# sdmiller/cpu_tsdf

Measured on NVIDIA H100. Metric: integrateCloud frames/s @ 640x480 into 2048^3, higher is better.
Workload: dtype f32

## Files before the change

cpu_tsdf_b200/csrc/brick_kernels.cuh:

```cuda
#pragma once
#include "tsdf_core.cuh"
#include "obs_fast.cuh"

namespace b2 {

struct QNode
{
  int x, y, z;
  int slot, idx;
  int kind;
  int child_base;
  int rc;
};

struct FrameRec
{
  Frame f;
  float pl[6][4];
  int cset;
  int timing;
  int pad_[2];
  unsigned long long kt[2];
};
__device__ __forceinline__ void pdl_launch_dependents () { asm volatile ("griddepcontrol.launch_dependents;" ::: "memory"); }
// ... 218 lines not shown
        Obs oc = observe (p, f, ch.cx, ch.cy, ch.cz, ch.size);
        rc = visit_fresh_leaf (p, f, ch, oc, cnt);
      }
      const unsigned nonneg = __ballot_sync (0xffffffffu, lane < 8 && rc >= 0);
      upd += cnt.n_updates; vis += cnt.n_visits;
      if (nonneg) return 1;
      if (lane == 0) atomicAnd (sw, ~m);
      if (lane < 8) reset_node (p, ch);
      __syncwarp ();
    }
  }
  int rc = 0;
  if (lane == 0) { bool updated; rc = leaf_update (p, f, n, o, updated); upd += updated; }
  return __shfl_sync (0xffffffffu, rc, 0);
}

constexpr int FRESH_RECS = 128;
struct CoopWarp
{
  __device__ __forceinline__ int lane () const { return threadIdx.x & 31; }
  __device__ __forceinline__ int nlanes () const { return 32; }
  __device__ __forceinline__ void sync () const { __syncwarp (); }
};
__device__ __noinline__ int leaf_visit_warp_bfs (const Params& p, const Frame& f, const NodePos& n, FreshRec* rec, int* counter,
                                                 unsigned long long& upd, unsigned long long& vis)
{
  const int lane = threadIdx.x & 31;
  Obs o = observe (p, f, n.cx, n.cy, n.cz, n.size);
  if (!o.valid) return 0;
  if (o.near_ && n.size > p.finest_size)
  {
    uint32_t m; uint32_t* sw = split_word (p, n, m);
    int cs = -1;
    if (lane == 0) cs = children_slot (p, n, true);
    cs = __shfl_sync (0xffffffffu, cs, 0);
    if (cs >= 0)
    {
      if (lane == 0) atomicOr (sw, m);
      __syncwarp ();
      Counters cnt; cnt.n_updates = 0; cnt.n_visits = 0;
      const bool stays = fresh_children_bfs (p, f, n, cs, rec, FRESH_RECS, counter, CoopWarp (), cnt);
      upd += cnt.n_updates; vis += cnt.n_visits;
      if (stays) return 1;
      if (lane == 0) atomicAnd (sw, ~m);
      if (lane < 8) reset_node (p, rec[lane].n);
      __syncwarp ();
    }
  }
  int rc = 0;
  if (lane == 0) { bool updated; rc = leaf_update (p, f, n, o, updated); upd += updated; }
  return __shfl_sync (0xffffffffu, rc, 0);
}

__device__ __noinline__ int leaf_visit_groups (const Params& p, const Frame& f, const NodePos& n, bool active,
                                               unsigned long long& upd, unsigned long long& vis)
{
  const int lane = threadIdx.x & 31, sub = lane & 7, g = lane >> 3;
  const unsigned gmask = 0xFFu << (8 * g);
  Obs o; o.valid = false; o.near_ = false; o.u = o.v = 0; o.d_new = 0.f;
  if (active) o = observe (p, f, n.cx, n.cy, n.cz, n.size);
  const bool live = active && o.valid;
  const bool want_split = live && o.near_ && n.size > p.finest_size;
  uint32_t m = 0; uint32_t* sw = nullptr;
  int cs = -1;
  if (want_split) { sw = split_word (p, n, m); if (sub == 0) cs = children_slot (p, n, true); }
  cs = __shfl_sync (0xffffffffu, cs, 8 * g);
  const bool split = want_split && cs >= 0;
  if (split && sub == 0) atomicOr (sw, m);
  __syncwarp ();
  Counters cnt; cnt.n_updates = 0; cnt.n_visits = 0;
  int crc = -1;
  NodePos ch = n;
  if (split)
  {
    ch = make_child (p, n, sub, cs);
    Obs oc = observe (p, f, ch.cx, ch.cy, ch.cz, ch.size);
    crc = visit_fresh_leaf (p, f, ch, oc, cnt);
  }
  const unsigned nonneg = __ballot_sync (0xffffffffu, split && crc >= 0) & gmask;
  upd += cnt.n_updates; vis += cnt.n_visits;
  if (split && !nonneg)
  {
    if (sub == 0) atomicAnd (sw, ~m);
    reset_node (p, ch);
  }
  __syncwarp ();
  int rc = 0;
  if (split && nonneg) rc = 1;
  else if (live && sub == 0) { bool updated; rc = leaf_update (p, f, n, o, updated); upd += updated; }
  return __shfl_sync (0xffffffffu, rc, 8 * g);
}
__device__ __forceinline__ void leaf_visit_slow_lanes (const Params& p, const Frame& f, bool slow, const NodePos& n, int t1, int& rc,
                                                       unsigned long long& upd, unsigned long long& vis)
{
  const int lane = threadIdx.x & 31, g = lane >> 3;
  uint32_t sm = __ballot_sync (0xffffffffu, slow);
  while (sm)
  {
    int srcs[4];
#pragma unroll
    for (int k = 0; k < 4; ++k) { srcs[k] = sm ? __ffs (sm) - 1 : -1; if (sm) sm &= sm - 1; }
    int src = srcs[0]; if (g == 1) src = srcs[1]; if (g == 2) src = srcs[2]; if (g == 3) src = srcs[3];
    const int from = src >= 0 ? src : 0;
    NodePos q;
    q.level = __shfl_sync (0xffffffffu, n.level, from); q.x = __shfl_sync (0xffffffffu, n.x, from); q.y = __shfl_sync (0xffffffffu, n.y, from); q.z = __shfl_sync (0xffffffffu, n.z, from);
    q.cx = __shfl_sync (0xffffffffu, n.cx, from); q.cy = __shfl_sync (0xffffffffu, n.cy, from); q.cz = __shfl_sync (0xffffffffu, n.cz, from);
    q.size = __shfl_sync (0xffffffffu, n.size, from); q.slot = t1; q.idx = __shfl_sync (0xffffffffu, n.idx, from);
    __threadfence_block ();
    const int r = leaf_visit_groups (p, f, q, src >= 0, upd, vis);
#pragma unroll
    for (int k = 0; k < 4; ++k) { const int rk = __shfl_sync (0xffffffffu, r, 8 * k); if (lane == srcs[k]) rc = rk; }
  }
}

__device__ __forceinline__ void path_center (const float* c0, float off, int k, int j, float* c)
{
  float x = c0[0], y = c0[1], z = c0[2];
  for (int l = k - 1; l >= 0; --l)
  {
    int cc = (j >> (3 * l)) & 7;
    x = (cc & 4) ? fadd (x, off) : fsub (x, off);
    y = (cc & 2) ? fadd (y, off) : fsub (y, off);
    z = (cc & 1) ? fadd (z, off) : fsub (z, off);
    off *= 0.5f;
  }
  c[0] = x; c[1] = y; c[2] = z;
}

constexpr int TOP_THREADS = 256;
constexpr int TOP_NODES = 585;
struct CellTop
{
  int t1slot, nblk;
  unsigned char kind[592];
  signed char rc[592];
  float dnew[73];
  int uv[73];
};
struct TopSmem
{
  float2 dw[BRICK_NODES];
  uchar4 rgb[BRICK_NODES];
  float o_dnew[TOP_NODES];
  int o_uv[TOP_NODES];
  uint32_t o_bgra[TOP_NODES];
  unsigned char o_flags[592];
  unsigned char kind[592];
  signed char rc[592];
  unsigned char dirty[592];
  uint32_t split[BRICK_SPLIT_WORDS];
  uint32_t split_old[BRICK_SPLIT_WORDS];
  QNode cell;
  int t1slot, root_interior;
  float c0[3];
};

__device__ __forceinline__ void top_kj (int f, int& k, int& j)
{ if (f == 0) { k = 0; j = 0; } else if (f < 9) { k = 1; j = f - 1; } else if (f < 73) { k = 2; j = f - 9; } else { k = 3; j = f - 73; } }

template <bool COLOR>
__global__ void __launch_bounds__ (TOP_THREADS) k_celltop_down (Params p, const FrameRec* __restrict__ fr, QNode* __restrict__ cells, int* __restrict__ d_count,
                                                               QNode* __restrict__ gq, CellTop* __restrict__ tops, int cell_cap,
                                                               int* __restrict__ blist, int bl_stride, unsigned long long* __restrict__ stats,
                                                               int SL, int qslot, int static_count)
{
  __shared__ __align__ (16) TopSmem S;
  __shared__ Frame s_f_;
  __shared__ float s_pl_[6][4];
  const int tid = threadIdx.x, lane = tid & 31;
  pdl_launch_dependents ();
  {
    const int* src_ = reinterpret_cast<const int*> (&fr->f); int* dst_ = reinterpret_cast<int*> (&s_f_);
    for (int w_ = tid; w_ < (int) (sizeof (Frame) / sizeof (int)); w_ += TOP_THREADS) dst_[w_] = src_[w_];
    if (tid < 24) s_pl_[tid >> 2][tid & 3] = fr->pl[tid >> 2][tid & 3];
  }
  int* const cnt_ = d_count + 16 * fr->cset;
  __syncthreads ();
  pdl_wait ();
  const Frame& f = s_f_;
  unsigned long long upd = 0, vis = 0;
  int count = qslot >= 0 ? cnt_[qslot] : static_count;
  if (count > cell_cap) { if (tid == 0 && blockIdx.x == 0) raise_err (p, ERR_QUEUE_FULL); count = cell_cap; }
  const int cell_lvl = p.C - SL;
  const float sizeC = level_size (p, SL);
  const float off1 = sizeC * 0.25f;
  const double thr[4] = { near_threshold (sizeC), near_threshold (sizeC * 0.5f), near_threshold (sizeC * 0.25f), near_threshold (sizeC * 0.125f) };
  const float thrf[4] = { float_at_least (thr[0]), float_at_least (thr[1]), float_at_least (thr[2]), float_at_least (thr[3]) };
// ... 29 lines not shown
      if (cell_lvl > 0)
      {
        kind = KIND_OLD;
        slot = find_brick (p, 1, cell.x, cell.y, cell.z);
        if (slot < 0) { raise_err (p, ERR_MISSING_BRICK); kind = KIND_DONE; }
      }
      else
      {
        NodePos nc; nc.level = SL; nc.x = cell.x; nc.y = cell.y; nc.z = cell.z; nc.cx = c0[0]; nc.cy = c0[1]; nc.cz = c0[2]; nc.size = sizeC; nc.slot = cell.slot; nc.idx = cell.idx;
        uint32_t m; uint32_t* sw = split_word (p, nc, m);
        vis++;
        if (*sw & m) { kind = KIND_OLD; slot = find_brick (p, 1, cell.x, cell.y, cell.z); if (slot < 0) { raise_err (p, ERR_MISSING_BRICK); kind = KIND_DONE; } }
        else
        {
          Obs o = observe_thr (p, f, c0[0], c0[1], c0[2], thr[0]);
          if (o.valid)
          {
            if (o.near_) { slot = find_or_insert_brick (p, 1, cell.x, cell.y, cell.z); if (slot >= 0) { kind = KIND_NEW; atomicOr (sw, m); } }
            else { bool u_; rc = leaf_update (p, f, nc, o, u_); upd += u_; }
          }
        }
        if (kind == KIND_DONE) cells[ci].rc = rc;
      }
      S.root_interior = kind; S.t1slot = slot;
      S.kind[0] = (unsigned char) kind; S.rc[0] = (signed char) rc;
    }
    __syncthreads ();
    const int t1 = S.t1slot;
    CellTop* top = tops + ci;
    if (S.root_interior == KIND_DONE)
    {
      if (tid == 0) { top->t1slot = -1; top->nblk = 0; top->kind[0] = KIND_DONE; top->rc[0] = S.rc[0]; }
      continue;
    }
    float2* gdw = p.nodes + (size_t) t1 * BRICK_NODES;
    uchar4* grgb = COLOR ? p.rgb + (size_t) t1 * BRICK_NODES : nullptr;
    uint32_t* gsw = p.split + (size_t) t1 * BRICK_SPLIT_WORDS;
    {
      const float4* g4 = reinterpret_cast<const float4*> (gdw);
      float4* s4 = reinterpret_cast<float4*> (S.dw);
      for (int i = tid; i < BRICK_NODES / 2; i += TOP_THREADS) s4[i] = g4[i];
      if (COLOR)
      {
        const uint4* gc = reinterpret_cast<const uint4*> (grgb);
        uint4* sc = reinterpret_cast<uint4*> (S.rgb);
        for (int i = tid; i < BRICK_NODES / 4; i += TOP_THREADS) sc[i] = gc[i];
// ... 68 lines not shown
          if (cls == c) blist[(size_t) c * bl_stride + b + __popc (mask & ((1u << lane) - 1))] = ci * STRIDE + 73 + j3;
        }
      }
    }
    for (int n = 1 + tid; n < TOP_NODES; n += TOP_THREADS)
      if (S.dirty[n]) { gdw[n - 1] = S.dw[n - 1]; if (COLOR) grgb[n - 1] = S.rgb[n - 1]; }
    if (tid < BRICK_SPLIT_WORDS && S.split[tid] != S.split_old[tid]) gsw[tid] = S.split[tid];
    for (int n = tid; n < 592; n += TOP_THREADS) { top->kind[n] = n < TOP_NODES ? S.kind[n] : 0; top->rc[n] = n < TOP_NODES ? S.rc[n] : 0; }
    for (int n = tid; n < 73; n += TOP_THREADS) { top->dnew[n] = S.o_dnew[n]; top->uv[n] = S.o_uv[n]; }
    if (tid == 0) { top->t1slot = t1; top->nblk = 0; }
  }
  __syncwarp ();
  warp_add_stats (stats, upd, vis);
}

__device__ __forceinline__ int top_fallthrough_new (const Params& p, const Frame& f, const NodePos& n, float dnew, int uv, unsigned long long& upd)
{
  Obs o; o.valid = true; o.near_ = true; o.d_new = dnew; o.u = uv & 0xFFFF; o.v = uv >> 16;
  bool u_; int rc = leaf_update (p, f, n, o, u_); upd += u_;
  return rc;
}

template <bool COLOR>
__global__ void __launch_bounds__ (128) k_celltop_up (Params gp, const FrameRec* __restrict__ fr, QNode* __restrict__ cells, const int* __restrict__ d_count,
                                                      const QNode* __restrict__ gq, const CellTop* __restrict__ tops, int cell_cap,
                                                      unsigned long long* __restrict__ stats, int SL, int qslot, int static_count)
{
  __shared__ Params sp_;
  __shared__ Frame sf_;
  __shared__ FreshRec s_rec[4][FRESH_RECS];
  __shared__ int s_cnt[4];
  pdl_launch_dependents ();
  {
    const int* s1 = reinterpret_cast<const int*> (&gp); int* d1 = reinterpret_cast<int*> (&sp_);
    for (int w = threadIdx.x; w < (int) (sizeof (Params) / sizeof (int)); w += blockDim.x) d1[w] = s1[w];
    const int* s2 = reinterpret_cast<const int*> (&fr->f); int* d2 = reinterpret_cast<int*> (&sf_);
    for (int w = threadIdx.x; w < (int) (sizeof (Frame) / sizeof (int)); w += blockDim.x) d2[w] = s2[w];
  }
  __syncthreads ();
  pdl_wait ();
  const Params& p = sp_;
  const Frame& f = sf_;
  const int lane = threadIdx.x & 31;
  const int warp = (blockIdx.x * blockDim.x + threadIdx.x) >> 5, nwarps = (gridDim.x * blockDim.x) >> 5;
  unsigned long long upd = 0, vis = 0;
  int count = qslot >= 0 ? d_count[16 * fr->cset + qslot] : static_count;
  if (count > cell_cap) count = cell_cap;
  if (fr->timing && blockIdx.x == 0 && threadIdx.x == 0 && fr->kt[1] > fr->kt[0])
  { atomicAdd (&stats[5], fr->kt[1] - fr->kt[0]); atomicAdd (&stats[6], 1ull); }
  const float sizeC = level_size (p, SL);
  const float off1 = sizeC * 0.25f;
  const int cell_lvl = p.C - SL;
  constexpr int STRIDE = 585;
  const long long c_entry = clock64 ();
  for (int ci = warp; ci < count; ci += nwarps)
  {
    const long long tc0 = clock64 ();
    int dbg_slow2 = 0, dbg_slow1 = 0, dbg_ft = 0;
    const CellTop* top = tops + ci;
    const int t1 = top->t1slot;
    if (t1 < 0) continue;
    const QNode cell = cells[ci];
    const float c0[3] = { center1d (p, SL, cell.x), center1d (p, SL, cell.y), center1d (p, SL, cell.z) };
    float2* gdw = p.nodes + (size_t) t1 * BRICK_NODES;
    uchar4* grgb = COLOR ? p.rgb + (size_t) t1 * BRICK_NODES : nullptr;
    uint32_t* gsw = p.split + (size_t) t1 * BRICK_SPLIT_WORDS;
    const int kind1 = lane < 8 ? top->kind[1 + lane] : KIND_DONE;
    int kind2[2]; kind2[0] = top->kind[9 + lane]; kind2[1] = top->kind[9 + 32 + lane];
    const uint32_t int1 = __ballot_sync (0xffffffffu, kind1 != KIND_DONE);
    uint32_t int2[2]; int2[0] = __ballot_sync (0xffffffffu, kind2[0] != KIND_DONE); int2[1] = __ballot_sync (0xffffffffu, kind2[1] != KIND_DONE);
    uint32_t nonneg_mine = 0;
    {
      int k3[16], r3[16];
#pragma unroll
      for (int i = 0; i < 16; ++i) { k3[i] = top->kind[73 + lane + 32 * i]; r3[i] = top->rc[73 + lane + 32 * i]; }
#pragma unroll
      for (int i = 0; i < 16; ++i) if (k3[i] != KIND_DONE) r3[i] = gq[(size_t) ci * STRIDE + 73 + lane + 32 * i].rc;
#pragma unroll
      for (int i = 0; i < 16; ++i)
      {
        const int j2 = (lane + 32 * i) >> 3;
        const bool visited = ((j2 < 32 ? int2[0] : int2[1]) >> (j2 & 31)) & 1;
        const uint32_t nn = __ballot_sync (0xffffffffu, visited && r3[i] >= 0);
        if (lane == i) nonneg_mine = nn;
      }
    }
    const long long cA = clock64 ();
    uint32_t nonneg2[2];
#pragma unroll
    for (int i2 = 0; i2 < 2; ++i2)
    {
      const int j2 = lane + 32 * i2;
      const uint32_t nn = __shfl_sync (0xffffffffu, nonneg_mine, (lane >> 2) + 8 * i2);
      int rc = top->rc[9 + j2];
      bool slow = false;
      NodePos n;
      if (kind2[i2] != KIND_DONE)
      {
        if (((nn >> (8 * (lane & 3))) & 0xFFu) != 0 || 2 < cell_lvl) rc = 1;
        else
        {
          atomicAnd (&gsw[1 + (j2 >> 5)], ~(1u << (j2 & 31)));
          for (int c = 0; c < 8; ++c) { gdw[72 + 8 * j2 + c] = make_float2 (-1.f, 0.f); if (COLOR) grgb[72 + 8 * j2 + c] = make_uchar4 (0, 0, 0, 0); }
          float c[3]; path_center (c0, off1, 2, j2, c);
          n.level = SL + 2; n.cx = c[0]; n.cy = c[1]; n.cz = c[2]; n.size = sizeC * 0.25f; n.slot = t1; n.idx = 8 + j2;
          { int lx = 0, ly = 0, lz = 0; for (int q = 1; q >= 0; --q) { int cc = (j2 >> (3 * q)) & 7; lx = (lx << 1) | (cc >> 2); ly = (ly << 1) | ((cc >> 1) & 1); lz = (lz << 1) | (cc & 1); }
            n.x = (cell.x << 2) | lx; n.y = (cell.y << 2) | ly; n.z = (cell.z << 2) | lz; }
          if (kind2[i2] == KIND_NEW) { rc = top_fallthrough_new (p, f, n, top->dnew[9 + j2], top->uv[9 + j2], upd); dbg_ft++; }
          else slow = true;
        }
      }
      dbg_slow2 += __popc (__ballot_sync (0xffffffffu, slow));
      leaf_visit_slow_lanes (p, f, slow, n, t1, rc, upd, vis);
      const bool visited2 = (int1 >> (j2 >> 3)) & 1;
      nonneg2[i2] = __ballot_sync (0xffffffffu, visited2 && rc >= 0);
    }
    const long long cB = clock64 ();
    int rc1 = lane < 8 ? (int) top->rc[1 + lane] : 0;
    {
      bool slow = false;
      NodePos n;
      if (lane < 8 && kind1 != KIND_DONE)
      {
        const uint32_t nn = nonneg2[lane >> 2];
        if (((nn >> (8 * (lane & 3))) & 0xFFu) != 0 || 1 < cell_lvl) rc1 = 1;
        else
        {
          atomicAnd (&gsw[0], ~(1u << lane));
          for (int c = 0; c < 8; ++c) { gdw[8 + 8 * lane + c] = make_float2 (-1.f, 0.f); if (COLOR) grgb[8 + 8 * lane + c] = make_uchar4 (0, 0, 0, 0); }
          float c[3]; path_center (c0, off1, 1, lane, c);
          n.level = SL + 1; n.cx = c[0]; n.cy = c[1]; n.cz = c[2]; n.size = sizeC * 0.5f; n.slot = t1; n.idx = lane;
          n.x = (cell.x << 1) | ((lane >> 2) & 1); n.y = (cell.y << 1) | ((lane >> 1) & 1); n.z = (cell.z << 1) | (lane & 1);
          if (kind1 == KIND_NEW) rc1 = top_fallthrough_new (p, f, n, top->dnew[1 + lane], top->uv[1 + lane], upd);
          else slow = true;
        }
      }
      dbg_slow1 += __popc (__ballot_sync (0xffffffffu, slow));
      leaf_visit_slow_lanes (p, f, slow, n, t1, rc1, upd, vis);
    }
    const uint32_t nonneg1 = __ballot_sync (0xffffffffu, lane < 8 && rc1 >= 0);
    const long long cC = clock64 ();
    int dbg_cell = 0;
    int rc_cell = 1;
    if ((nonneg1 & 0xFFu) == 0 && cell_lvl <= 0)
    {
      dbg_cell = top->kind[0] == KIND_NEW ? 1 : 2;
      NodePos nc; nc.level = SL; nc.x = cell.x; nc.y = cell.y; nc.z = cell.z; nc.cx = c0[0]; nc.cy = c0[1]; nc.cz = c0[2]; nc.size = sizeC; nc.slot = cell.slot; nc.idx = cell.idx;
      if (lane == 0) { uint32_t m; uint32_t* sw = split_word (p, nc, m); atomicAnd (sw, ~m); }
      if (lane < 8) { gdw[lane] = make_float2 (-1.f, 0.f); if (COLOR) grgb[lane] = make_uchar4 (0, 0, 0, 0); }
      __syncwarp ();
      if (top->kind[0] == KIND_NEW) { if (lane == 0) rc_cell = top_fallthrough_new (p, f, nc, top->dnew[0], top->uv[0], upd); rc_cell = __shfl_sync (0xffffffffu, rc_cell, 0); }
      else { __threadfence_block (); rc_cell = leaf_visit_warp_bfs (p, f, nc, s_rec[threadIdx.x >> 5], &s_cnt[threadIdx.x >> 5], upd, vis); }
    }
    if (lane == 0 && cell_lvl <= 0) cells[ci].rc = rc_cell;
    if (p.dbg && lane == 0)
    {
      const long long cD = clock64 ();
      const unsigned long long tag = ((unsigned long long) (dbg_slow2 & 0xFF) << 24) | ((unsigned long long) (dbg_slow1 & 0xF) << 20) | ((unsigned long long) (dbg_cell & 3) << 18) | (unsigned long long) (ci & 0x3FFFF);
      atomicMax (&p.dbg[0], ((unsigned long long) (cD - tc0) << 32) | tag);
      atomicMax (&p.dbg[1], ((unsigned long long) (cA - tc0) << 32) | tag);
      atomicMax (&p.dbg[2], ((unsigned long long) (cB - cA) << 32) | tag);
      atomicMax (&p.dbg[3], ((unsigned long long) (cC - cB) << 32) | tag);
      atomicMax (&p.dbg[4], ((unsigned long long) (cD - cC) << 32) | tag);
      atomicMax (&p.dbg[5], ((unsigned long long) (tc0 - c_entry) << 32) | tag);
      atomicAdd (&p.dbg[6], (unsigned long long) dbg_slow2); atomicAdd (&p.dbg[7], (unsigned long long) dbg_slow1);
      atomicAdd (&p.dbg[8], (unsigned long long) (dbg_cell == 2)); atomicAdd (&p.dbg[9], (unsigned long long) (dbg_cell == 1));
      atomicAdd (&p.dbg[10], 1ull);
    }
  }
  __syncwarp ();
  warp_add_stats (stats, upd, vis);
}

}
```

cpu_tsdf_b200/csrc/engine.cu:

```cuda
#include "../../include/b200tsdf.h"
#include "tsdf_core.cuh"
#include "mc_tables.cuh"
#include "host_math.h"
#include "params_setup.h"
#include "brick_kernels.cuh"
#include "brick_direct.cuh"
#include "organize.cuh"
#include "mesh_sort.h"
#include "host_pack.h"

#include <cuda_runtime.h>
#include <sys/mman.h>
#include <sys/syscall.h>
#include <unistd.h>
#include <algorithm>
#include <cstdio>
#include <cstdlib>
#include <cstring>
#include <string>
#include <type_traits>
#include <unordered_map>
#include <vector>

using namespace b2;
// ... 477 lines not shown
  b200tsdf_config cfg_pending{}, cfg{};
  bool has_volume = false;
  Params p{};
  int device = 0, sm_count = 0;
  cudaStream_t stream = nullptr, copy_stream = nullptr, gather_stream = nullptr;
  size_t pool = 0;
  bool alloc_color = false, alloc_var = false, alloc_norm = false;
  size_t root_n = 0;
  int* d_err = nullptr;
  unsigned char* d_frame[2] = { nullptr, nullptr };
  size_t frame_cap = 0;
  cudaEvent_t ev_copied[2] = { nullptr, nullptr }, ev_consumed[2] = { nullptr, nullptr };
  cudaEvent_t ev_t0 = nullptr, ev_t1 = nullptr, ev_k0 = nullptr, ev_k1 = nullptr;
  uint64_t frame_no = 0;
  int count_set = 0;
  int* d_culled = nullptr; int* d_count = nullptr; unsigned long long* d_stats = nullptr;
  size_t culled_cap = 0;
  bool timed = false;
  bool time_frames = false;
  bool is_empty = true;
  Queues Q{}; int q_levels = 0; QNode* q_mem = nullptr; size_t q_mem_cap = 0;
  int* d_blist = nullptr; int* d_bail = nullptr; size_t blist_cap = 0;
  int cell_cap = 0; QNode* d_cellq = nullptr; size_t cellq_cap = 0; CellTop* d_celltop = nullptr; QNode* d_superq = nullptr;
  bool top_path = false, replayable = false; int sl = 0, nup = 0, super_static = 0;
  bool fast_path = false; int force_general = 0;
  bool use_pdl = true;
  int bd_minb = 6;
  Params* d_params = nullptr;
  unsigned long long* d_dbg = nullptr;
  int* h_err = nullptr;
  FrameRec* d_ring = nullptr; FrameRec* h_ring = nullptr; uint64_t ring_seq = 0;
  cudaEvent_t ev_ring[2] = { nullptr, nullptr };
  FrameRec* d_bring = nullptr; FrameRec* h_bring = nullptr; int bring_half = 0; int bring_seg = 0; bool bring_used[BATCH_SEGS] = {};
  cudaEvent_t ev_bring[BATCH_SEGS] = {};
  cudaEvent_t ev_half_done[2] = { nullptr, nullptr }; bool half_used[2] = { false, false }; FrameRec* batch_recs = nullptr;
  cudaGraphExec_t batch_exec[2][FRAME_RING / 2 + 1] = {};
  void* comm = nullptr; int comm_rank = 0, comm_size = 1;
  unsigned char* d_rows_raw[2] = { nullptr, nullptr }; unsigned char* d_rows_full[2] = { nullptr, nullptr };
  size_t rows_raw_cap = 0, rows_full_cap = 0; int rows_set = 0; bool rows_used[2] = { false, false }; int rows_last_up[2] = { 0, 0 };
  int rows_chunk = 0;
  cudaEvent_t ev_rows_up[2][32] = {}, ev_rows_ready[2][32] = {}, ev_rows_done[2] = { nullptr, nullptr };
  int host_pack = -1;
  int pack_threads = 0;
  b2host::PackPool* pack_pool = nullptr;
  Staging h_pack[2]; size_t pack_cap = 0;
  Staging h_fpack[2];
// ... 217 lines not shown
  if (!h) return;
  cudaSetDevice (h->device);
  if (h->stream) cudaStreamSynchronize (h->stream);
  if (h->copy_stream) cudaStreamSynchronize (h->copy_stream);
  if (h->gather_stream) cudaStreamSynchronize (h->gather_stream);
  free_volume (h);
  cudaFree (h->d_err); cudaFree (h->d_count); cudaFree (h->d_stats); cudaFree (h->d_culled); cudaFree (h->d_scratch);
  cudaFree (h->d_dbg); if (h->h_err) cudaFreeHost (h->h_err);
  cudaFree (h->d_params); cudaFree (h->d_ring); if (h->h_ring) cudaFreeHost (h->h_ring);
  for (int i = 0; i < 2; ++i) if (h->ev_ring[i]) cudaEventDestroy (h->ev_ring[i]);
  drop_batch_graphs (h);
  comm_release (h);
  delete h->pack_pool; h->pack_pool = nullptr;
  for (int i = 0; i < 2; ++i)
  {
    cudaFree (h->d_rows_raw[i]); cudaFree (h->d_rows_full[i]);
    h->h_pack[i].release (); h->h_fpack[i].release ();
    for (int k = 0; k < 32; ++k) { if (h->ev_rows_ready[i][k]) cudaEventDestroy (h->ev_rows_ready[i][k]); if (h->ev_rows_up[i][k]) cudaEventDestroy (h->ev_rows_up[i][k]); }
    if (h->ev_rows_done[i]) cudaEventDestroy (h->ev_rows_done[i]);
  }
  cudaFree (h->d_bring); if (h->h_bring) cudaFreeHost (h->h_bring);
  for (int i = 0; i < BATCH_SEGS; ++i) if (h->ev_bring[i]) cudaEventDestroy (h->ev_bring[i]);
  for (int i = 0; i < 2; ++i) if (h->ev_half_done[i]) cudaEventDestroy (h->ev_half_done[i]);
  cudaFree (h->d_frame[0]); cudaFree (h->d_frame[1]); cudaFree (h->q_mem); cudaFree (h->d_blist); cudaFree (h->d_bail); cudaFree (h->d_cellq); cudaFree (h->d_superq); cudaFree (h->d_celltop);
  for (int i = 0; i < 2; ++i) { if (h->ev_copied[i]) cudaEventDestroy (h->ev_copied[i]); if (h->ev_consumed[i]) cudaEventDestroy (h->ev_consumed[i]); }
  if (h->ev_t0) cudaEventDestroy (h->ev_t0); if (h->ev_t1) cudaEventDestroy (h->ev_t1);
  if (h->ev_k0) cudaEventDestroy (h->ev_k0); if (h->ev_k1) cudaEventDestroy (h->ev_k1);
  if (h->ev_p0) cudaEventDestroy (h->ev_p0); if (h->ev_p1) cudaEventDestroy (h->ev_p1);
  for (int i = 0; i < KRING; ++i) { if (h->kring[i][0]) cudaEventDestroy (h->kring[i][0]); if (h->kring[i][1]) cudaEventDestroy (h->kring[i][1]); }
  if (h->stream) cudaStreamDestroy (h->stream);
  if (h->copy_stream) cudaStreamDestroy (h->copy_stream);
  if (h->gather_stream) cudaStreamDestroy (h->gather_stream);
  std::free (h->mesh_v); std::free (h->mesh_c); std::free (h->leaf_xyz); std::free (h->leaf_ijk);
  delete h;
}

const char* b200tsdf_last_error (const b200tsdf_t* h) { return h ? h->err.c_str () : "null handle"; }

int b200tsdf_set_config (b200tsdf_t* h, const b200tsdf_config* cfg)
{
  if (!h || !cfg) return B200TSDF_EINVAL;
  int dev = h->cfg_pending.device;
  h->cfg_pending = *cfg;
  h->cfg_pending.device = dev;
  std::memcpy (h->cfg.global_transform, cfg->global_transform, sizeof (h->cfg.global_transform));
  return B200TSDF_OK;
}
// ... 63 lines not shown
      cudaFree (h->q_mem); h->q_mem = nullptr; h->q_mem_cap = 0;
      CK (cudaMalloc (&h->q_mem, total * sizeof (QNode)));
      h->q_mem_cap = total;
    }
    size_t off = 0;
    for (int i = 0; i < MAX_QLEVELS; ++i) { h->Q.q[i] = nullptr; h->Q.cap[i] = 0; }
    for (int i = 0; i < h->q_levels; ++i) { h->Q.q[i] = h->q_mem + off; h->Q.cap[i] = (int) caps[i]; off += caps[i]; }
    h->Q.n = h->d_count;
    h->sl = np.L - 6;
    h->nup = std::max (0, h->sl - np.C);
    h->super_static = 0;
    h->top_path = h->fast_path && np.T >= 2 && h->sl >= 0 && !(c.debug_flags & 6);
    if (h->top_path && np.C > h->sl)
    {
      if (np.Rtop != h->sl || h->sl > 4) h->top_path = false;
      else h->super_static = 1 << (3 * h->sl);
    }
    if (h->top_path)
    {
      h->cell_cap = 16384;
      size_t need = (size_t) h->cell_cap * 585;
      if (need > h->cellq_cap)
      {
        cudaFree (h->d_cellq); cudaFree (h->d_celltop); h->d_cellq = nullptr; h->d_celltop = nullptr; h->cellq_cap = 0;
        CK (cudaMalloc (&h->d_cellq, need * sizeof (QNode)));
        CK (cudaMalloc (&h->d_celltop, (size_t) h->cell_cap * sizeof (CellTop)));
        h->cellq_cap = need;
      }
      if (h->super_static && !h->d_superq) CK (cudaMalloc (&h->d_superq, 4096 * sizeof (QNode)));
    }
    h->replayable = h->fast_path;
    size_t bl = h->q_levels ? caps[h->q_levels - 1] : 0;
    if (h->top_path) bl = std::max (bl, (size_t) h->cell_cap * 512);
    if (bl > h->blist_cap)
    {
      cudaFree (h->d_blist); cudaFree (h->d_bail); h->d_blist = h->d_bail = nullptr; h->blist_cap = 0;
      CK (cudaMalloc (&h->d_blist, bl * BL_CLASSES * sizeof (int)));
      CK (cudaMalloc (&h->d_bail, bl * sizeof (int)));
      h->blist_cap = bl;
    }
  }
  Params& p = h->p;
  {
    Params st = p;
    p = np;
    p.work = st.work;
    p.keys = st.keys; p.nodes = st.nodes; p.split = st.split; p.rgb = st.rgb; p.M = st.M; p.ns = st.ns;
    p.root_dw = st.root_dw; p.root_split = st.root_split; p.root_rgb = st.root_rgb; p.root_M = st.root_M; p.root_ns = st.root_ns;
    p.rgbn = st.rgbn; p.root_rgbn = st.root_rgbn;
// ... 53 lines not shown
  {
    const int cull_blocks = (ncells + 255) / 256;
    const bool pdl = h->replayable && h->use_pdl;
    if (pdl) CK (launch_pdl (k_front, dim3 (cull_blocks + (npix + 255) / 256), dim3 (256), s, p, d_rec, cull_blocks, h->d_culled, h->d_count, h->Q.q[0], h->d_stats));
    else k_front<<<cull_blocks + (npix + 255) / 256, 256, 0, s>>> (p, d_rec, cull_blocks, h->d_culled, h->d_count, h->fast_path ? h->Q.q[0] : nullptr, h->d_stats);
  }
  h->launches += 1;
  int kr = -1;
  if (with_events)
  {
    if (h->kring_pending >= KRING) h->drain_kring (KRING / 2);
    kr = h->kring_head;
  }
  if (h->fast_path)
  {
    const int nl = h->q_levels;
    QNode* bq = nullptr;
    if (h->top_path)
    {
      for (int li = 0; li < h->nup; ++li) { k_upper_down<<<h->sm_count * 2, 128, 0, s>>> (p, d_rec, h->Q, li, 0, h->d_blist, h->d_stats); h->launches++; }
      QNode* cells = h->super_static ? h->d_superq : h->Q.q[h->nup];
      const int qslot = h->super_static ? -1 : h->nup;
      auto kd = p.color ? k_celltop_down<true> : k_celltop_down<false>;
      if (h->use_pdl) CK (launch_pdl (kd, dim3 (h->sm_count * 4), dim3 (TOP_THREADS), s, p, d_rec, cells, h->d_count, h->d_cellq, h->d_celltop, h->cell_cap, h->d_blist, (int) h->blist_cap, h->d_stats, h->sl, qslot, h->super_static));
      else kd<<<h->sm_count * 4, TOP_THREADS, 0, s>>> (p, d_rec, cells, h->d_count, h->d_cellq, h->d_celltop, h->cell_cap, h->d_blist, (int) h->blist_cap, h->d_stats, h->sl, qslot, h->super_static);
      h->launches++;
      bq = h->d_cellq;
    }
    else
    {
      for (int li = 0; li < nl; ++li) { k_upper_down<<<h->sm_count * 2, 128, 0, s>>> (p, d_rec, h->Q, li, li == nl - 1, h->d_blist, h->d_stats); h->launches++; }
      bq = h->Q.q[nl - 1];
    }
    if (kr >= 0) CK (cudaEventRecord (h->kring[kr][0], s));
    {
      auto kb = h->bd_minb == 6 ? (p.color ? k_bricks<true, 6> : k_bricks<false, 6>) : (p.color ? k_bricks<true, 8> : k_bricks<false, 8>);
      const dim3 g (h->sm_count * h->bd_minb), b (BD_WARPS * 32);
      if (h->top_path && h->use_pdl) CK (launch_pdl (kb, g, b, s, p, (const Params*) h->d_params, d_rec, bq, (const int*) h->d_blist, (int) h->blist_cap, h->d_count, h->d_stats, p.L - 3));
      else kb<<<g, b, 0, s>>> (p, h->d_params, d_rec, bq, h->d_blist, (int) h->blist_cap, h->d_count, h->d_stats, p.L - 3);
    }
    if (kr >= 0) CK (cudaEventRecord (h->kring[kr][1], s));
    h->launches++;
    if (h->top_path)
    {
      QNode* cells = h->super_static ? h->d_superq : h->Q.q[h->nup];
      const int qslot = h->super_static ? -1 : h->nup;
      auto ku = p.color ? k_celltop_up<true> : k_celltop_up<false>;
      if (h->use_pdl) CK (launch_pdl (ku, dim3 (h->sm_count), dim3 (128), s, p, d_rec, cells, (const int*) h->d_count, (const QNode*) h->d_cellq, (const CellTop*) h->d_celltop, h->cell_cap, h->d_stats, h->sl, qslot, h->super_static));
      else ku<<<h->sm_count, 128, 0, s>>> (p, d_rec, cells, h->d_count, h->d_cellq, h->d_celltop, h->cell_cap, h->d_stats, h->sl, qslot, h->super_static);
      h->launches++;
      for (int li = h->nup - 1; li >= 0; --li) { k_upper_up<<<h->sm_count * 2, 128, 0, s>>> (p, d_rec, h->Q, li, h->d_stats); h->launches++; }
    }
    else
      for (int li = nl - 2; li >= 0; --li) { k_upper_up<<<h->sm_count * 2, 128, 0, s>>> (p, d_rec, h->Q, li, h->d_stats); h->launches++; }
  }
  else
  {
    if (kr >= 0) CK (cudaEventRecord (h->kring[kr][0], s));
    k_update_dfs<<<(ncells + 31) / 32, 32, 0, s>>> (p, f, h->d_culled, cnt, h->d_stats);
    if (kr >= 0) CK (cudaEventRecord (h->kring[kr][1], s));
    h->launches++;
  }
  if (kr >= 0) { h->kring_head = (kr + 1) % KRING; h->kring_pending++; }
  h->prof_frames++;
  return B200TSDF_OK;
}

static int ring_slot (b200tsdf* h, int& slot)
{
  slot = (int) (h->ring_seq % FRAME_RING);
  const int half = FRAME_RING / 2;
  if (h->ring_seq >= (uint64_t) FRAME_RING && slot % half == 0) CK (cudaEventSynchronize (h->ev_ring[slot / half]));
// ... 1140 lines not shown
```

Measured before the change: 9606.

## Compact active top cells into a list and process each with a whole CTA

The down kernel now appends the index of every cell that is not done to a compacted toplist through an atomic counter. The up kernel walks that list with one 128-thread block per cell instead of one warp per cell over all cells. Inside a cell it spreads level-3 and level-2 work across threads, collects slow nodes into shared queues, and runs them with a templated BFS that uses the whole block when there is a single slow node. This aims to remove idle warps on finished cells and serialized slow lanes, at the cost of more __syncthreads per cell and an extra atomic and list write in the down kernel.

```diff
diff --git a/cpu_tsdf_b200/csrc/brick_kernels.cuh b/cpu_tsdf_b200/csrc/brick_kernels.cuh
--- a/cpu_tsdf_b200/csrc/brick_kernels.cuh
+++ b/cpu_tsdf_b200/csrc/brick_kernels.cuh
@@ -264,95 +264,44 @@
   __device__ __forceinline__ int nlanes () const { return 32; }
   __device__ __forceinline__ void sync () const { __syncwarp (); }
 };
-__device__ __noinline__ int leaf_visit_warp_bfs (const Params& p, const Frame& f, const NodePos& n, FreshRec* rec, int* counter,
-                                                 unsigned long long& upd, unsigned long long& vis)
-{
-  const int lane = threadIdx.x & 31;
+struct CoopBlock
+{
+  __device__ __forceinline__ int lane () const { return threadIdx.x; }
+  __device__ __forceinline__ int nlanes () const { return blockDim.x; }
+  __device__ __forceinline__ void sync () const { __syncthreads (); }
+};
+template <typename Coop>
+__device__ __noinline__ int leaf_visit_bfs (const Params& p, const Frame& f, const NodePos& n, FreshRec* rec, int cap, int* counter,
+                                            const Coop& co, unsigned long long& upd, unsigned long long& vis)
+{
+  const int lane = co.lane ();
   Obs o = observe (p, f, n.cx, n.cy, n.cz, n.size);
   if (!o.valid) return 0;
   if (o.near_ && n.size > p.finest_size)
   {
     uint32_t m; uint32_t* sw = split_word (p, n, m);
-    int cs = -1;
-    if (lane == 0) cs = children_slot (p, n, true);
-    cs = __shfl_sync (0xffffffffu, cs, 0);
+    if (lane == 0) *counter = children_slot (p, n, true);
+    co.sync ();
+    const int cs = *counter;
+    co.sync ();
     if (cs >= 0)
     {
       if (lane == 0) atomicOr (sw, m);
-      __syncwarp ();
+      co.sync ();
       Counters cnt; cnt.n_updates = 0; cnt.n_visits = 0;
-      const bool stays = fresh_children_bfs (p, f, n, cs, rec, FRESH_RECS, counter, CoopWarp (), cnt);
+      const bool stays = fresh_children_bfs (p, f, n, cs, rec, cap, counter, co, cnt);
       upd += cnt.n_updates; vis += cnt.n_visits;
       if (stays) return 1;
       if (lane == 0) atomicAnd (sw, ~m);
-      if (lane < 8) reset_node (p, rec[lane].n);
-      __syncwarp ();
-    }
-  }
-  int rc = 0;
-  if (lane == 0) { bool updated; rc = leaf_update (p, f, n, o, updated); upd += updated; }
-  return __shfl_sync (0xffffffffu, rc, 0);
-}
-
-__device__ __noinline__ int leaf_visit_groups (const Params& p, const Frame& f, const NodePos& n, bool active,
-                                               unsigned long long& upd, unsigned long long& vis)
-{
-  const int lane = threadIdx.x & 31, sub = lane & 7, g = lane >> 3;
-  const unsigned gmask = 0xFFu << (8 * g);
-  Obs o; o.valid = false; o.near_ = false; o.u = o.v = 0; o.d_new = 0.f;
-  if (active) o = observe (p, f, n.cx, n.cy, n.cz, n.size);
-  const bool live = active && o.valid;
-  const bool want_split = live && o.near_ && n.size > p.finest_size;
-  uint32_t m = 0; uint32_t* sw = nullptr;
-  int cs = -1;
-  if (want_split) { sw = split_word (p, n, m); if (sub == 0) cs = children_slot (p, n, true); }
-  cs = __shfl_sync (0xffffffffu, cs, 8 * g);
-  const bool split = want_split && cs >= 0;
-  if (split && sub == 0) atomicOr (sw, m);
-  __syncwarp ();
-  Counters cnt; cnt.n_updates = 0; cnt.n_visits = 0;
-  int crc = -1;
-  NodePos ch = n;
-  if (split)
-  {
-    ch = make_child (p, n, sub, cs);
-    Obs oc = observe (p, f, ch.cx, ch.cy, ch.cz, ch.size);
-    crc = visit_fresh_leaf (p, f, ch, oc, cnt);
-  }
-  const unsigned nonneg = __ballot_sync (0xffffffffu, split && crc >= 0) & gmask;
-  upd += cnt.n_updates; vis += cnt.n_visits;
-  if (split && !nonneg)
-  {
-    if (sub == 0) atomicAnd (sw, ~m);
-    reset_node (p, ch);
-  }
-  __syncwarp ();
-  int rc = 0;
-  if (split && nonneg) rc = 1;
-  else if (live && sub == 0) { bool updated; rc = leaf_update (p, f, n, o, updated); upd += updated; }
-  return __shfl_sync (0xffffffffu, rc, 8 * g);
-}
-__device__ __forceinline__ void leaf_visit_slow_lanes (const Params& p, const Frame& f, bool slow, const NodePos& n, int t1, int& rc,
-                                                       unsigned long long& upd, unsigned long long& vis)
-{
-  const int lane = threadIdx.x & 31, g = lane >> 3;
-  uint32_t sm = __ballot_sync (0xffffffffu, slow);
-  while (sm)
-  {
-    int srcs[4];
-#pragma unroll
-    for (int k = 0; k < 4; ++k) { srcs[k] = sm ? __ffs (sm) - 1 : -1; if (sm) sm &= sm - 1; }
-    int src = srcs[0]; if (g == 1) src = srcs[1]; if (g == 2) src = srcs[2]; if (g == 3) src = srcs[3];
-    const int from = src >= 0 ? src : 0;
-    NodePos q;
-    q.level = __shfl_sync (0xffffffffu, n.level, from); q.x = __shfl_sync (0xffffffffu, n.x, from); q.y = __shfl_sync (0xffffffffu, n.y, from); q.z = __shfl_sync (0xffffffffu, n.z, from);
-    q.cx = __shfl_sync (0xffffffffu, n.cx, from); q.cy = __shfl_sync (0xffffffffu, n.cy, from); q.cz = __shfl_sync (0xffffffffu, n.cz, from);
-    q.size = __shfl_sync (0xffffffffu, n.size, from); q.slot = t1; q.idx = __shfl_sync (0xffffffffu, n.idx, from);
-    __threadfence_block ();
-    const int r = leaf_visit_groups (p, f, q, src >= 0, upd, vis);
-#pragma unroll
-    for (int k = 0; k < 4; ++k) { const int rk = __shfl_sync (0xffffffffu, r, 8 * k); if (lane == srcs[k]) rc = rk; }
-  }
+      for (int c = lane; c < 8; c += co.nlanes ()) reset_node (p, rec[c].n);
+      co.sync ();
+    }
+  }
+  if (lane == 0) { bool updated; *counter = leaf_update (p, f, n, o, updated); upd += updated; }
+  co.sync ();
+  const int rc = *counter;
+  co.sync ();
+  return rc;
 }
 
 __device__ __forceinline__ void path_center (const float* c0, float off, int k, int j, float* c)
@@ -370,6 +319,8 @@
 }
 
 constexpr int TOP_THREADS = 256;
+constexpr int TOP_UP_THREADS = 128;
+constexpr int TOP_LIST_SLOT = 15;
 constexpr int TOP_NODES = 585;
 struct CellTop
 {
@@ -403,8 +354,8 @@
 template <bool COLOR>
 __global__ void __launch_bounds__ (TOP_THREADS) k_celltop_down (Params p, const FrameRec* __restrict__ fr, QNode* __restrict__ cells, int* __restrict__ d_count,
                                                                QNode* __restrict__ gq, CellTop* __restrict__ tops, int cell_cap,
-                                                               int* __restrict__ blist, int bl_stride, unsigned long long* __restrict__ stats,
-                                                               int SL, int qslot, int static_count)
+                                                               int* __restrict__ blist, int bl_stride, int* __restrict__ toplist,
+                                                               unsigned long long* __restrict__ stats, int SL, int qslot, int static_count)
 {
   __shared__ __align__ (16) TopSmem S;
   __shared__ Frame s_f_;
@@ -480,6 +431,7 @@
         }
         if (kind == KIND_DONE) cells[ci].rc = rc;
       }
+      if (kind != KIND_DONE) toplist[atomicAdd (cnt_ + TOP_LIST_SLOT, 1)] = ci;
       S.root_interior = kind; S.t1slot = slot;
       S.kind[0] = (unsigned char) kind; S.rc[0] = (signed char) rc;
     }
@@ -594,14 +546,18 @@
 }
 
 template <bool COLOR>
-__global__ void __launch_bounds__ (128) k_celltop_up (Params gp, const FrameRec* __restrict__ fr, QNode* __restrict__ cells, const int* __restrict__ d_count,
-                                                      const QNode* __restrict__ gq, const CellTop* __restrict__ tops, int cell_cap,
-                                                      unsigned long long* __restrict__ stats, int SL, int qslot, int static_count)
-{
+__global__ void __launch_bounds__ (TOP_UP_THREADS) k_celltop_up (Params gp, const FrameRec* __restrict__ fr, QNode* __restrict__ cells, const int* __restrict__ d_count,
+                                                                 const int* __restrict__ toplist, const QNode* __restrict__ gq, const CellTop* __restrict__ tops,
+                                                                 unsigned long long* __restrict__ stats, int SL)
+{
+  constexpr int NWARPS = TOP_UP_THREADS / 32;
   __shared__ Params sp_;
   __shared__ Frame sf_;
-  __shared__ FreshRec s_rec[4][FRESH_RECS];
-  __shared__ int s_cnt[4];
+  __shared__ FreshRec s_rec[NWARPS * FRESH_RECS];
+  __shared__ int s_cnt[NWARPS];
+  __shared__ signed char s_rc2[64], s_rc1[8];
+  __shared__ unsigned char s_slow2[64], s_slow1[8];
+  __shared__ int s_nslow2, s_nslow1;
   pdl_launch_dependents ();
   {
     const int* s1 = reinterpret_cast<const int*> (&gp); int* d1 = reinterpret_cast<int*> (&sp_);
@@ -613,129 +569,148 @@
   pdl_wait ();
   const Params& p = sp_;
   const Frame& f = sf_;
-  const int lane = threadIdx.x & 31;
-  const int warp = (blockIdx.x * blockDim.x + threadIdx.x) >> 5, nwarps = (gridDim.x * blockDim.x) >> 5;
+  const int tid = threadIdx.x, lane = tid & 31, warp = tid >> 5;
   unsigned long long upd = 0, vis = 0;
-  int count = qslot >= 0 ? d_count[16 * fr->cset + qslot] : static_count;
-  if (count > cell_cap) count = cell_cap;
-  if (fr->timing && blockIdx.x == 0 && threadIdx.x == 0 && fr->kt[1] > fr->kt[0])
+  const int count = d_count[16 * fr->cset + TOP_LIST_SLOT];
+  if (fr->timing && blockIdx.x == 0 && tid == 0 && fr->kt[1] > fr->kt[0])
   { atomicAdd (&stats[5], fr->kt[1] - fr->kt[0]); atomicAdd (&stats[6], 1ull); }
   const float sizeC = level_size (p, SL);
   const float off1 = sizeC * 0.25f;
   const int cell_lvl = p.C - SL;
   constexpr int STRIDE = 585;
   const long long c_entry = clock64 ();
-  for (int ci = warp; ci < count; ci += nwarps)
+  for (int li = blockIdx.x; li < count; li += gridDim.x)
   {
     const long long tc0 = clock64 ();
-    int dbg_slow2 = 0, dbg_slow1 = 0, dbg_ft = 0;
+    const int ci = toplist[li];
     const CellTop* top = tops + ci;
     const int t1 = top->t1slot;
-    if (t1 < 0) continue;
     const QNode cell = cells[ci];
     const float c0[3] = { center1d (p, SL, cell.x), center1d (p, SL, cell.y), center1d (p, SL, cell.z) };
     float2* gdw = p.nodes + (size_t) t1 * BRICK_NODES;
     uchar4* grgb = COLOR ? p.rgb + (size_t) t1 * BRICK_NODES : nullptr;
     uint32_t* gsw = p.split + (size_t) t1 * BRICK_SPLIT_WORDS;
-    const int kind1 = lane < 8 ? top->kind[1 + lane] : KIND_DONE;
-    int kind2[2]; kind2[0] = top->kind[9 + lane]; kind2[1] = top->kind[9 + 32 + lane];
-    const uint32_t int1 = __ballot_sync (0xffffffffu, kind1 != KIND_DONE);
-    uint32_t int2[2]; int2[0] = __ballot_sync (0xffffffffu, kind2[0] != KIND_DONE); int2[1] = __ballot_sync (0xffffffffu, kind2[1] != KIND_DONE);
-    uint32_t nonneg_mine = 0;
-    {
-      int k3[16], r3[16];
+    if (tid == 0) { s_nslow2 = 0; s_nslow1 = 0; }
+    __syncthreads ();
+    const int j2 = tid >> 1;
+    bool nonneg3 = false;
+    {
+      const int j3 = 8 * j2 + 4 * (tid & 1);
+      int k3[4], r3[4];
 #pragma unroll
-      for (int i = 0; i < 16; ++i) { k3[i] = top->kind[73 + lane + 32 * i]; r3[i] = top->rc[73 + lane + 32 * i]; }
+      for (int c = 0; c < 4; ++c) { k3[c] = top->kind[73 + j3 + c]; r3[c] = top->rc[73 + j3 + c]; }
 #pragma unroll
-      for (int i = 0; i < 16; ++i) if (k3[i] != KIND_DONE) r3[i] = gq[(size_t) ci * STRIDE + 73 + lane + 32 * i].rc;
+      for (int c = 0; c < 4; ++c) if (k3[c] != KIND_DONE) r3[c] = gq[(size_t) ci * STRIDE + 73 + j3 + c].rc;
 #pragma unroll
-      for (int i = 0; i < 16; ++i)
-      {
-        const int j2 = (lane + 32 * i) >> 3;
-        const bool visited = ((j2 < 32 ? int2[0] : int2[1]) >> (j2 & 31)) & 1;
-        const uint32_t nn = __ballot_sync (0xffffffffu, visited && r3[i] >= 0);
-        if (lane == i) nonneg_mine = nn;
-      }
+      for (int c = 0; c < 4; ++c) nonneg3 |= r3[c] >= 0;
+      nonneg3 |= __shfl_xor_sync (0xffffffffu, nonneg3, 1);
     }
     const long long cA = clock64 ();
-    uint32_t nonneg2[2];
-#pragma unroll
-    for (int i2 = 0; i2 < 2; ++i2)
-    {
-      const int j2 = lane + 32 * i2;
-      const uint32_t nn = __shfl_sync (0xffffffffu, nonneg_mine, (lane >> 2) + 8 * i2);
+    if ((tid & 1) == 0)
+    {
+      const int kind2 = top->kind[9 + j2];
       int rc = top->rc[9 + j2];
-      bool slow = false;
-      NodePos n;
-      if (kind2[i2] != KIND_DONE)
-      {
-        if (((nn >> (8 * (lane & 3))) & 0xFFu) != 0 || 2 < cell_lvl) rc = 1;
+      if (kind2 != KIND_DONE)
+      {
+        if (nonneg3 || 2 < cell_lvl) rc = 1;
         else
         {
           atomicAnd (&gsw[1 + (j2 >> 5)], ~(1u << (j2 & 31)));
           for (int c = 0; c < 8; ++c) { gdw[72 + 8 * j2 + c] = make_float2 (-1.f, 0.f); if (COLOR) grgb[72 + 8 * j2 + c] = make_uchar4 (0, 0, 0, 0); }
-          float c[3]; path_center (c0, off1, 2, j2, c);
-          n.level = SL + 2; n.cx = c[0]; n.cy = c[1]; n.cz = c[2]; n.size = sizeC * 0.25f; n.slot = t1; n.idx = 8 + j2;
-          { int lx = 0, ly = 0, lz = 0; for (int q = 1; q >= 0; --q) { int cc = (j2 >> (3 * q)) & 7; lx = (lx << 1) | (cc >> 2); ly = (ly << 1) | ((cc >> 1) & 1); lz = (lz << 1) | (cc & 1); }
-            n.x = (cell.x << 2) | lx; n.y = (cell.y << 2) | ly; n.z = (cell.z << 2) | lz; }
-          if (kind2[i2] == KIND_NEW) { rc = top_fallthrough_new (p, f, n, top->dnew[9 + j2], top->uv[9 + j2], upd); dbg_ft++; }
-          else slow = true;
+          if (kind2 == KIND_NEW)
+          {
+            float c[3]; path_center (c0, off1, 2, j2, c);
+            NodePos n; n.level = SL + 2; n.cx = c[0]; n.cy = c[1]; n.cz = c[2]; n.size = sizeC * 0.25f; n.slot = t1; n.idx = 8 + j2;
+            { int lx = 0, ly = 0, lz = 0; for (int q = 1; q >= 0; --q) { int cc = (j2 >> (3 * q)) & 7; lx = (lx << 1) | (cc >> 2); ly = (ly << 1) | ((cc >> 1) & 1); lz = (lz << 1) | (cc & 1); }
+              n.x = (cell.x << 2) | lx; n.y = (cell.y << 2) | ly; n.z = (cell.z << 2) | lz; }
+            rc = top_fallthrough_new (p, f, n, top->dnew[9 + j2], top->uv[9 + j2], upd);
+          }
+          else s_slow2[atomicAdd (&s_nslow2, 1)] = (unsigned char) j2;
         }
       }
-      dbg_slow2 += __popc (__ballot_sync (0xffffffffu, slow));
-      leaf_visit_slow_lanes (p, f, slow, n, t1, rc, upd, vis);
-      const bool visited2 = (int1 >> (j2 >> 3)) & 1;
-      nonneg2[i2] = __ballot_sync (0xffffffffu, visited2 && rc >= 0);
-    }
+      s_rc2[j2] = (signed char) rc;
+    }
+    __syncthreads ();
+    const int nslow2 = s_nslow2;
+    for (int s = nslow2 == 1 ? 0 : warp; s < nslow2; s += NWARPS)
+    {
+      const int j = s_slow2[s];
+      float c[3]; path_center (c0, off1, 2, j, c);
+      NodePos n; n.level = SL + 2; n.cx = c[0]; n.cy = c[1]; n.cz = c[2]; n.size = sizeC * 0.25f; n.slot = t1; n.idx = 8 + j;
+      { int lx = 0, ly = 0, lz = 0; for (int q = 1; q >= 0; --q) { int cc = (j >> (3 * q)) & 7; lx = (lx << 1) | (cc >> 2); ly = (ly << 1) | ((cc >> 1) & 1); lz = (lz << 1) | (cc & 1); }
+        n.x = (cell.x << 2) | lx; n.y = (cell.y << 2) | ly; n.z = (cell.z << 2) | lz; }
+      const int r = nslow2 == 1 ? leaf_visit_bfs (p, f, n, s_rec, NWARPS * FRESH_RECS, &s_cnt[0], CoopBlock (), upd, vis)
+                                : leaf_visit_bfs (p, f, n, s_rec + warp * FRESH_RECS, FRESH_RECS, &s_cnt[warp], CoopWarp (), upd, vis);
+      if (lane == 0) s_rc2[j] = (signed char) r;
+    }
+    __syncthreads ();
     const long long cB = clock64 ();
-    int rc1 = lane < 8 ? (int) top->rc[1 + lane] : 0;
-    {
-      bool slow = false;
-      NodePos n;
-      if (lane < 8 && kind1 != KIND_DONE)
-      {
-        const uint32_t nn = nonneg2[lane >> 2];
-        if (((nn >> (8 * (lane & 3))) & 0xFFu) != 0 || 1 < cell_lvl) rc1 = 1;
+    if (tid < 8)
+    {
+      const int kind1 = top->kind[1 + tid];
+      int rc = top->rc[1 + tid];
+      if (kind1 != KIND_DONE)
+      {
+        bool nonneg2 = false;
+        for (int c = 0; c < 8; ++c) nonneg2 |= s_rc2[8 * tid + c] >= 0;
+        if (nonneg2 || 1 < cell_lvl) rc = 1;
         else
         {
-          atomicAnd (&gsw[0], ~(1u << lane));
-          for (int c = 0; c < 8; ++c) { gdw[8 + 8 * lane + c] = make_float2 (-1.f, 0.f); if (COLOR) grgb[8 + 8 * lane + c] = make_uchar4 (0, 0, 0, 0); }
-          float c[3]; path_center (c0, off1, 1, lane, c);
-          n.level = SL + 1; n.cx = c[0]; n.cy = c[1]; n.cz = c[2]; n.size = sizeC * 0.5f; n.slot = t1; n.idx = lane;
-          n.x = (cell.x << 1) | ((lane >> 2) & 1); n.y = (cell.y << 1) | ((lane >> 1) & 1); n.z = (cell.z << 1) | (lane & 1);
-          if (kind1 == KIND_NEW) rc1 = top_fallthrough_new (p, f, n, top->dnew[1 + lane], top->uv[1 + lane], upd);
-          else slow = true;
+          atomicAnd (&gsw[0], ~(1u << tid));
+          for (int c = 0; c < 8; ++c) { gdw[8 + 8 * tid + c] = make_float2 (-1.f, 0.f); if (COLOR) grgb[8 + 8 * tid + c] = make_uchar4 (0, 0, 0, 0); }
+          if (kind1 == KIND_NEW)
+          {
+            float c[3]; path_center (c0, off1, 1, tid, c);
+            NodePos n; n.level = SL + 1; n.cx = c[0]; n.cy = c[1]; n.cz = c[2]; n.size = sizeC * 0.5f; n.slot = t1; n.idx = tid;
+            n.x = (cell.x << 1) | ((tid >> 2) & 1); n.y = (cell.y << 1) | ((tid >> 1) & 1); n.z = (cell.z << 1) | (tid & 1);
+            rc = top_fallthrough_new (p, f, n, top->dnew[1 + tid], top->uv[1 + tid], upd);
+          }
+          else s_slow1[atomicAdd (&s_nslow1, 1)] = (unsigned char) tid;
         }
       }
-      dbg_slow1 += __popc (__ballot_sync (0xffffffffu, slow));
-      leaf_visit_slow_lanes (p, f, slow, n, t1, rc1, upd, vis);
-    }
-    const uint32_t nonneg1 = __ballot_sync (0xffffffffu, lane < 8 && rc1 >= 0);
+      s_rc1[tid] = (signed char) rc;
+    }
+    __syncthreads ();
+    const int nslow1 = s_nslow1;
+    for (int s = nslow1 == 1 ? 0 : warp; s < nslow1; s += NWARPS)
+    {
+      const int j = s_slow1[s];
+      float c[3]; path_center (c0, off1, 1, j, c);
+      NodePos n; n.level = SL + 1; n.cx = c[0]; n.cy = c[1]; n.cz = c[2]; n.size = sizeC * 0.5f; n.slot = t1; n.idx = j;
+      n.x = (cell.x << 1) | ((j >> 2) & 1); n.y = (cell.y << 1) | ((j >> 1) & 1); n.z = (cell.z << 1) | (j & 1);
+      const int r = nslow1 == 1 ? leaf_visit_bfs (p, f, n, s_rec, NWARPS * FRESH_RECS, &s_cnt[0], CoopBlock (), upd, vis)
+                                : leaf_visit_bfs (p, f, n, s_rec + warp * FRESH_RECS, FRESH_RECS, &s_cnt[warp], CoopWarp (), upd, vis);
+      if (lane == 0) s_rc1[j] = (signed char) r;
+    }
+    __syncthreads ();
     const long long cC = clock64 ();
+    bool nonneg1 = false;
+    for (int c = 0; c < 8; ++c) nonneg1 |= s_rc1[c] >= 0;
     int dbg_cell = 0;
     int rc_cell = 1;
-    if ((nonneg1 & 0xFFu) == 0 && cell_lvl <= 0)
-    {
-      dbg_cell = top->kind[0] == KIND_NEW ? 1 : 2;
+    if (!nonneg1 && cell_lvl <= 0)
+    {
+      const int kind0 = top->kind[0];
+      dbg_cell = kind0 == KIND_NEW ? 1 : 2;
       NodePos nc; nc.level = SL; nc.x = cell.x; nc.y = cell.y; nc.z = cell.z; nc.cx = c0[0]; nc.cy = c0[1]; nc.cz = c0[2]; nc.size = sizeC; nc.slot = cell.slot; nc.idx = cell.idx;
-      if (lane == 0) { uint32_t m; uint32_t* sw = split_word (p, nc, m); atomicAnd (sw, ~m); }
-      if (lane < 8) { gdw[lane] = make_float2 (-1.f, 0.f); if (COLOR) grgb[lane] = make_uchar4 (0, 0, 0, 0); }
-      __syncwarp ();
-      if (top->kind[0] == KIND_NEW) { if (lane == 0) rc_cell = top_fallthrough_new (p, f, nc, top->dnew[0], top->uv[0], upd); rc_cell = __shfl_sync (0xffffffffu, rc_cell, 0); }
-      else { __threadfence_block (); rc_cell = leaf_visit_warp_bfs (p, f, nc, s_rec[threadIdx.x >> 5], &s_cnt[threadIdx.x >> 5], upd, vis); }
-    }
-    if (lane == 0 && cell_lvl <= 0) cells[ci].rc = rc_cell;
-    if (p.dbg && lane == 0)
+      if (tid == 0) { uint32_t m; uint32_t* sw = split_word (p, nc, m); atomicAnd (sw, ~m); }
+      if (tid < 8) { gdw[tid] = make_float2 (-1.f, 0.f); if (COLOR) grgb[tid] = make_uchar4 (0, 0, 0, 0); }
+      __syncthreads ();
+      if (kind0 == KIND_NEW) { if (tid == 0) rc_cell = top_fallthrough_new (p, f, nc, top->dnew[0], top->uv[0], upd); }
+      else rc_cell = leaf_visit_bfs (p, f, nc, s_rec, NWARPS * FRESH_RECS, &s_cnt[0], CoopBlock (), upd, vis);
+    }
+    if (tid == 0 && cell_lvl <= 0) cells[ci].rc = rc_cell;
+    if (p.dbg && tid == 0)
     {
       const long long cD = clock64 ();
-      const unsigned long long tag = ((unsigned long long) (dbg_slow2 & 0xFF) << 24) | ((unsigned long long) (dbg_slow1 & 0xF) << 20) | ((unsigned long long) (dbg_cell & 3) << 18) | (unsigned long long) (ci & 0x3FFFF);
+      const unsigned long long tag = ((unsigned long long) (nslow2 & 0xFF) << 24) | ((unsigned long long) (nslow1 & 0xF) << 20) | ((unsigned long long) (dbg_cell & 3) << 18) | (unsigned long long) (ci & 0x3FFFF);
       atomicMax (&p.dbg[0], ((unsigned long long) (cD - tc0) << 32) | tag);
       atomicMax (&p.dbg[1], ((unsigned long long) (cA - tc0) << 32) | tag);
       atomicMax (&p.dbg[2], ((unsigned long long) (cB - cA) << 32) | tag);
       atomicMax (&p.dbg[3], ((unsigned long long) (cC - cB) << 32) | tag);
       atomicMax (&p.dbg[4], ((unsigned long long) (cD - cC) << 32) | tag);
       atomicMax (&p.dbg[5], ((unsigned long long) (tc0 - c_entry) << 32) | tag);
-      atomicAdd (&p.dbg[6], (unsigned long long) dbg_slow2); atomicAdd (&p.dbg[7], (unsigned long long) dbg_slow1);
+      atomicAdd (&p.dbg[6], (unsigned long long) nslow2); atomicAdd (&p.dbg[7], (unsigned long long) nslow1);
       atomicAdd (&p.dbg[8], (unsigned long long) (dbg_cell == 2)); atomicAdd (&p.dbg[9], (unsigned long long) (dbg_cell == 1));
       atomicAdd (&p.dbg[10], 1ull);
     }
diff --git a/cpu_tsdf_b200/csrc/engine.cu b/cpu_tsdf_b200/csrc/engine.cu
--- a/cpu_tsdf_b200/csrc/engine.cu
+++ b/cpu_tsdf_b200/csrc/engine.cu
@@ -523,6 +523,7 @@
   Queues Q{}; int q_levels = 0; QNode* q_mem = nullptr; size_t q_mem_cap = 0;
   int* d_blist = nullptr; int* d_bail = nullptr; size_t blist_cap = 0;
   int cell_cap = 0; QNode* d_cellq = nullptr; size_t cellq_cap = 0; CellTop* d_celltop = nullptr; QNode* d_superq = nullptr;
+  int* d_toplist = nullptr;
   bool top_path = false, replayable = false; int sl = 0, nup = 0, super_static = 0;
   bool fast_path = false; int force_general = 0;
   bool use_pdl = true;
@@ -786,7 +787,7 @@
   cudaFree (h->d_bring); if (h->h_bring) cudaFreeHost (h->h_bring);
   for (int i = 0; i < BATCH_SEGS; ++i) if (h->ev_bring[i]) cudaEventDestroy (h->ev_bring[i]);
   for (int i = 0; i < 2; ++i) if (h->ev_half_done[i]) cudaEventDestroy (h->ev_half_done[i]);
-  cudaFree (h->d_frame[0]); cudaFree (h->d_frame[1]); cudaFree (h->q_mem); cudaFree (h->d_blist); cudaFree (h->d_bail); cudaFree (h->d_cellq); cudaFree (h->d_superq); cudaFree (h->d_celltop);
+  cudaFree (h->d_frame[0]); cudaFree (h->d_frame[1]); cudaFree (h->q_mem); cudaFree (h->d_blist); cudaFree (h->d_bail); cudaFree (h->d_cellq); cudaFree (h->d_superq); cudaFree (h->d_celltop); cudaFree (h->d_toplist);
   for (int i = 0; i < 2; ++i) { if (h->ev_copied[i]) cudaEventDestroy (h->ev_copied[i]); if (h->ev_consumed[i]) cudaEventDestroy (h->ev_consumed[i]); }
   if (h->ev_t0) cudaEventDestroy (h->ev_t0); if (h->ev_t1) cudaEventDestroy (h->ev_t1);
   if (h->ev_k0) cudaEventDestroy (h->ev_k0); if (h->ev_k1) cudaEventDestroy (h->ev_k1);
@@ -896,9 +897,10 @@
       size_t need = (size_t) h->cell_cap * 585;
       if (need > h->cellq_cap)
       {
-        cudaFree (h->d_cellq); cudaFree (h->d_celltop); h->d_cellq = nullptr; h->d_celltop = nullptr; h->cellq_cap = 0;
+        cudaFree (h->d_cellq); cudaFree (h->d_celltop); cudaFree (h->d_toplist); h->d_cellq = nullptr; h->d_celltop = nullptr; h->d_toplist = nullptr; h->cellq_cap = 0;
         CK (cudaMalloc (&h->d_cellq, need * sizeof (QNode)));
         CK (cudaMalloc (&h->d_celltop, (size_t) h->cell_cap * sizeof (CellTop)));
+        CK (cudaMalloc (&h->d_toplist, (size_t) h->cell_cap * sizeof (int)));
         h->cellq_cap = need;
       }
       if (h->super_static && !h->d_superq) CK (cudaMalloc (&h->d_superq, 4096 * sizeof (QNode)));
@@ -998,8 +1000,8 @@
       QNode* cells = h->super_static ? h->d_superq : h->Q.q[h->nup];
       const int qslot = h->super_static ? -1 : h->nup;
       auto kd = p.color ? k_celltop_down<true> : k_celltop_down<false>;
-      if (h->use_pdl) CK (launch_pdl (kd, dim3 (h->sm_count * 4), dim3 (TOP_THREADS), s, p, d_rec, cells, h->d_count, h->d_cellq, h->d_celltop, h->cell_cap, h->d_blist, (int) h->blist_cap, h->d_stats, h->sl, qslot, h->super_static));
-      else kd<<<h->sm_count * 4, TOP_THREADS, 0, s>>> (p, d_rec, cells, h->d_count, h->d_cellq, h->d_celltop, h->cell_cap, h->d_blist, (int) h->blist_cap, h->d_stats, h->sl, qslot, h->super_static);
+      if (h->use_pdl) CK (launch_pdl (kd, dim3 (h->sm_count * 4), dim3 (TOP_THREADS), s, p, d_rec, cells, h->d_count, h->d_cellq, h->d_celltop, h->cell_cap, h->d_blist, (int) h->blist_cap, h->d_toplist, h->d_stats, h->sl, qslot, h->super_static));
+      else kd<<<h->sm_count * 4, TOP_THREADS, 0, s>>> (p, d_rec, cells, h->d_count, h->d_cellq, h->d_celltop, h->cell_cap, h->d_blist, (int) h->blist_cap, h->d_toplist, h->d_stats, h->sl, qslot, h->super_static);
       h->launches++;
       bq = h->d_cellq;
     }
@@ -1020,10 +1022,10 @@
     if (h->top_path)
     {
       QNode* cells = h->super_static ? h->d_superq : h->Q.q[h->nup];
-      const int qslot = h->super_static ? -1 : h->nup;
       auto ku = p.color ? k_celltop_up<true> : k_celltop_up<false>;
-      if (h->use_pdl) CK (launch_pdl (ku, dim3 (h->sm_count), dim3 (128), s, p, d_rec, cells, (const int*) h->d_count, (const QNode*) h->d_cellq, (const CellTop*) h->d_celltop, h->cell_cap, h->d_stats, h->sl, qslot, h->super_static));
-      else ku<<<h->sm_count, 128, 0, s>>> (p, d_rec, cells, h->d_count, h->d_cellq, h->d_celltop, h->cell_cap, h->d_stats, h->sl, qslot, h->super_static);
+      const int up_ctas = h->sm_count * 2;
+      if (h->use_pdl) CK (launch_pdl (ku, dim3 (up_ctas), dim3 (TOP_UP_THREADS), s, p, d_rec, cells, (const int*) h->d_count, (const int*) h->d_toplist, (const QNode*) h->d_cellq, (const CellTop*) h->d_celltop, h->d_stats, h->sl));
+      else ku<<<up_ctas, TOP_UP_THREADS, 0, s>>> (p, d_rec, cells, h->d_count, h->d_toplist, h->d_cellq, h->d_celltop, h->d_stats, h->sl);
       h->launches++;
       for (int li = h->nup - 1; li >= 0; --li) { k_upper_up<<<h->sm_count * 2, 128, 0, s>>> (p, d_rec, h->Q, li, h->d_stats); h->launches++; }
     }
```

After: 9788 (median of 6 runs). +1.9%, better.
